# tensorflow/recommenders

Measured on NVIDIA H100. Metric: queries/sec brute-force top-K (1Mx64 candidates), higher is better.
Workload: dtype f32 (fp16 wgmma screening, fp32 accumulate + exact fp32 re-scoring)

## Files before the change

### include/tfrs_b200.h

```cpp
#ifndef TFRS_B200_H_
#define TFRS_B200_H_

#include <stddef.h>
#include <stdint.h>

#ifdef __cplusplus
extern "C" {
#endif

#define TFRS_B200_VERSION 102

enum {
  TFRS_OK = 0,
  TFRS_ERR_INVALID_ARG = -1,
  TFRS_ERR_UNSUPPORTED = -2,
  TFRS_ERR_CUDA = -3,
  TFRS_ERR_WORKSPACE_TOO_SMALL = -4,
  TFRS_ERR_NCCL = -5
};

enum { TFRS_I32 = 0, TFRS_I64 = 1 };

int tfrs_version(void);
const char* tfrs_last_error(void);
// ... 26 lines not shown
                           void* stream);

int tfrs_topk_exclude_rerank_f32(const float* scores, const int64_t* idx, int64_t Q, int k_fetched,
                                 const int64_t* identifiers, const int64_t* exclusions, int n_excl, int k_out,
                                 float* out_scores, int64_t* out_idx, void* stream);

int tfrs_count_above_f32(const float* scores, int64_t ld, int k, const float* positive_scores, int64_t Q,
                         int32_t* out_count, void* stream);

int tfrs_topk_hits_accumulate(const int32_t* count, const float* positive_scores, const float* sample_weight, int64_t Q,
                              const int32_t* ks, int n_ks, double* acc, void* stream);

int tfrs_topk_tc_layout(int64_t Q, int64_t N, int d, int k, int64_t* out10);

int tfrs_topk_tc_retry_layout(int64_t Q, int64_t N, int d, int k, int64_t* out4);

int tfrs_profile_enable(int on);
int tfrs_profile_read(float* stage_ms, int* calls);

int tfrs_topk_merge_strided(const float* scores, const int64_t* idx, int64_t list_stride_scores,
                            int64_t list_stride_idx, int n_lists, int64_t Q, int k_in, int k_out,
                            float* out_scores, int64_t* out_idx, void* stream);

int tfrs_topk_merge_sorted_strided(const float* scores, const int64_t* idx, int64_t list_stride_scores,
                                   int64_t list_stride_idx, int n_lists, int64_t Q, int k_in, int k_out,
                                   float* out_scores, int64_t* out_idx, void* stream);

typedef struct tfrs_comm* tfrs_comm_t;
int tfrs_comm_unique_id(void* out128);
int tfrs_comm_create(tfrs_comm_t* comm, int rank, int world, const void* unique_id128);
// ... 235 lines not shown
```

### recommenders_b200/_ffi.py

```python
from __future__ import annotations

import ctypes
import os
from typing import Optional

import torch

_HERE = os.path.dirname(os.path.abspath(__file__))
LIB_PATH = os.environ.get("TFRS_B200_LIB", os.path.join(_HERE, "libtfrs_b200.so"))

_lib: Optional[ctypes.CDLL] = None

I32, I64, BYTES = 0, 1, 2
c_p = ctypes.c_void_p
c_i = ctypes.c_int
c_l = ctypes.c_int64
c_f = ctypes.c_float
c_sz = ctypes.c_size_t
c_u32 = ctypes.c_uint32

_SIGNATURES = {
    "tfrs_version": (c_i, []),
    "tfrs_last_error": (ctypes.c_char_p, []),
    "tfrs_launch_count": (c_l, []),
    "tfrs_gather_f32": (c_i, [c_p, c_p, c_p, c_i, c_p, c_i, c_l, c_p, c_l, c_p, c_p]),
    "tfrs_topk_scan_workspace_bytes": (c_sz, [c_l, c_l, c_i, c_i]),
    "tfrs_topk_scan_f32": (c_i, [c_p, c_l, c_p, c_l, c_i, c_i, c_l, c_p, c_p, c_i, c_p, c_p, c_p, c_sz, c_p]),
    "tfrs_index_bytes": (c_sz, [c_l, c_i]),
    "tfrs_index_build": (c_i, [c_p, c_l, c_i, c_p, c_sz, c_p]),
    "tfrs_topk_tc_workspace_bytes": (c_sz, [c_l, c_l, c_i, c_i]),
    "tfrs_topk_tc_f32": (c_i, [c_p, c_l, c_p, c_p, c_l, c_i, c_i, c_l, c_p, c_p, c_p, c_sz, c_p]),
    "tfrs_topk_tc_exclude_f32": (c_i, [c_p, c_l, c_p, c_p, c_l, c_i, c_i, c_l, c_p, c_p, c_i, c_p, c_p, c_p, c_sz, c_p]),
    "tfrs_topk_tc_count_f32": (c_i, [c_p, c_l, c_p, c_p, c_l, c_i, c_i, c_p, c_p, c_p, c_sz, c_p]),
    "tfrs_topk_exclude_rerank_f32": (c_i, [c_p, c_p, c_l, c_i, c_p, c_p, c_i, c_i, c_p, c_p, c_p]),
    "tfrs_count_above_f32": (c_i, [c_p, c_l, c_i, c_p, c_l, c_p, c_p]),
    "tfrs_topk_hits_accumulate": (c_i, [c_p, c_p, c_p, c_l, c_p, c_i, c_p, c_p]),
    "tfrs_topk_tc_layout": (c_i, [c_l, c_l, c_i, c_i, c_p]),
    "tfrs_topk_tc_retry_layout": (c_i, [c_l, c_l, c_i, c_i, c_p]),
    "tfrs_dot_interaction_out_dim": (c_i, [c_i, c_i, c_i]),
    "tfrs_dot_interaction_fwd_f32": (c_i, [c_p, c_l, c_i, c_i, c_i, c_i, c_p, c_p]),
    "tfrs_dot_interaction_bwd_f32": (c_i, [c_p, c_p, c_l, c_i, c_i, c_i, c_i, c_p, c_p]),
    "tfrs_profile_enable": (c_i, [c_i]),
    "tfrs_profile_read": (c_i, [c_p, c_p]),
    "tfrs_topk_merge_strided": (c_i, [c_p, c_p, c_l, c_l, c_i, c_l, c_i, c_i, c_p, c_p, c_p]),
    "tfrs_topk_merge_sorted_strided": (c_i, [c_p, c_p, c_l, c_l, c_i, c_l, c_i, c_i, c_p, c_p, c_p]),
    "tfrs_comm_unique_id": (c_i, [c_p]),
    "tfrs_comm_create": (c_i, [c_p, c_i, c_i, c_p]),
    "tfrs_comm_destroy": (c_i, [c_p]),
    "tfrs_comm_enable_p2p": (c_i, [c_p, c_l, c_i]),
    "tfrs_comm_p2p_capacity": (c_i, [c_p, c_l, c_i]),
    "tfrs_comm_set_option": (c_i, [c_p, c_i, c_i]),
    "tfrs_comm_rank": (c_i, [c_p]),
    "tfrs_comm_world": (c_i, [c_p]),
# ... 165 lines not shown
```

### recommenders_b200/csrc/topk_tc.cu

```cuda
#include <cuda_fp16.h>
#include <math.h>
#include <stdlib.h>
#include <type_traits>
#include "rowselect.cuh"
#include "tc_ptx.cuh"

namespace tfrs {
namespace tc {

constexpr int TILE_N = 128;
constexpr int TILE_M = 128;
constexpr int QBLK = 256;
constexpr int KSLAB = 64;
constexpr int SLAB_BYTES = TILE_N * 128;
constexpr int HEADER_BYTES = 1024;
constexpr int THREADS = 512;
constexpr int CONSUMER_WARPS = 16;
constexpr int CAND_CAP = 2048;
constexpr int MAX_SAMPLE_STRIDE = 4;
constexpr int FIN_MAX_PARTS = 2 * 132;
constexpr int MAX_BINS = 1024;
constexpr int FP16_TARGET = 15;
constexpr float E_REL = 0.00108f;
constexpr float E_ACC = 0.00013f;

struct SideStats {
  unsigned int max_norm2_bits;
  unsigned int amax_bits;
  int exp;
  int pad;
};
struct IndexHeader {
  SideStats st;
  int d, d_pad, kb, pad;
  long long n, n_tiles;
};

__device__ __forceinline__ int rescale_exp(float amax) {
  int x = 0;
  if (!(amax > 0.f) || !(amax < INFINITY)) return 0;
  (void)frexpf(amax, &x);
  return FP16_TARGET - x;
}

__global__ void __launch_bounds__(256)
tile_image_kernel(const float* __restrict__ src, long long rows, int d, int kb, long long n_tiles,
                  const SideStats* __restrict__ st, unsigned char* __restrict__ img) {
  const int scale_exp = st->exp;
  const long long total = n_tiles * TILE_N * (long long)kb * 8;
  for (long long e = (long long)blockIdx.x * 256 + threadIdx.x; e < total; e += (long long)gridDim.x * 256) {
    int chunk = (int)(e % (kb * 8));
    long long row = e / (kb * 8);
    int slab = chunk / 8, cj = chunk % 8;
    int r = (int)(row % TILE_N);
    long long tile = row / TILE_N;
    int k0 = slab * KSLAB + cj * 8;
    __align__(16) __half v[8];
#pragma unroll
    for (int j = 0; j < 8; ++j) {
      float f = (row < rows && k0 + j < d) ? src[row * d + k0 + j] : 0.f;
      v[j] = __float2half_rn(ldexpf(f, scale_exp));
    }
    unsigned char* dst = img + tile * ((long long)kb * SLAB_BYTES) + (long long)slab * SLAB_BYTES + r * 128 + ((cj ^ (r & 7)) * 16);
    *reinterpret_cast<uint4*>(dst) = *reinterpret_cast<const uint4*>(v);
  }
}

template <int PASS>
__global__ void __launch_bounds__(256)
corpus_stats_kernel(const float* __restrict__ src, long long rows, int d, SideStats* __restrict__ st) {
  const int lane = threadIdx.x & 31;
  const long long warp = ((long long)blockIdx.x * 256 + threadIdx.x) >> 5;
  const long long nwarps = ((long long)gridDim.x * 256) >> 5;
  const int e = PASS ? st->exp : 0;
  float best = 0.f;
  for (long long row = warp; row < rows; row += nwarps) {
    const float* p = src + row * d;
    float acc = 0.f;
    for (int k = lane; k < d; k += 32) {
      const float x = p[k];
      if (PASS) { const float y = ldexpf(x, e); acc = fmaf(y, y, acc); } else acc = fmaxf(acc, fabsf(x));
    }
#pragma unroll
    for (int o = 16; o > 0; o >>= 1) {
      const float other = __shfl_xor_sync(0xffffffffu, acc, o);
      acc = PASS ? acc + other : fmaxf(acc, other);
    }
    best = fmaxf(best, acc);
  }
  if (lane == 0 && best > 0.f) {
    if (PASS) atomicMax(&st->max_norm2_bits, __float_as_uint(best * 1.0001f));
    else atomicMax(&st->amax_bits, __float_as_uint(best));
  }
}
__global__ void side_exp_kernel(SideStats* st) { st->exp = rescale_exp(__uint_as_float(st->amax_bits)); }
__global__ void header_kernel(IndexHeader* dst, IndexHeader h) { *dst = h; }

__global__ void __launch_bounds__(256)
tc_qprep_kernel(const float* __restrict__ q, long long Q, long long Qp, int d, int kb, const IndexHeader* __restrict__ hdr,
                unsigned char* __restrict__ qimg, float* __restrict__ margin, float* __restrict__ cut, int* __restrict__ qexp) {
  const int lane = threadIdx.x & 31;
  const long long row = ((long long)blockIdx.x * 256 + threadIdx.x) >> 5;
  if (row >= Qp) return;
  const bool real = row < Q;
  const float* p = q + row * d;
  float a = 0.f;
  if (real) for (int k = lane; k < d; k += 32) a = fmaxf(a, fabsf(p[k]));
#pragma unroll
  for (int o = 16; o > 0; o >>= 1) a = fmaxf(a, __shfl_xor_sync(0xffffffffu, a, o));
  const int e = rescale_exp(a);
  float n2 = 0.f;
// ... 29 lines not shown
enum { FILTER_FULL = 0, FILTER_NO_EMIT = 1, FILTER_NO_EPILOGUE = 2 };
#if defined(TFRS_DEBUG_SWITCHES) && defined(TFRS_FILTER_ABLATION)
constexpr int FILTER_ABLATION = TFRS_FILTER_ABLATION;
#else
constexpr int FILTER_ABLATION = FILTER_FULL;
#endif

struct ScanParams {
  const unsigned char* qimg;
  const unsigned char* cimg;
  long long Q, N;
  int nqb, parts, n_seq, stride;
  long long n_tiles;
  float* binmax; int bins_ld;
  int group, bins_per_part;
  const float* thr;
  const unsigned int* retry;
  unsigned int* count;
  float* cand_s;
  unsigned int* cand_i;
  int cap_part;
};

template <int KB, int STAGES, int MODE>
__global__ void __launch_bounds__(THREADS, 1)
tc_scan_kernel(const ScanParams p) {
  extern __shared__ __align__(1024) unsigned char smem_raw[];
  unsigned char* smem = reinterpret_cast<unsigned char*>((reinterpret_cast<uintptr_t>(smem_raw) + 1023) & ~uintptr_t(1023));
  unsigned char* sA = smem;
  unsigned char* sB = smem + 2 * KB * SLAB_BYTES;
  uint64_t* bars = reinterpret_cast<uint64_t*>(sB + STAGES * KB * SLAB_BYTES);
  uint64_t* full = bars;
  uint64_t* empty = bars + STAGES;
  uint64_t* a_full = bars + 2 * STAGES;

  const int wg = threadIdx.x >> 7, warp = (threadIdx.x >> 5) & 3, lane = threadIdx.x & 31;
  const int qb = blockIdx.x % p.nqb, part = blockIdx.x / p.nqb;
  const int u_begin = (int)((long long)part * p.n_seq / p.parts);
  const int u_end = (int)((long long)(part + 1) * p.n_seq / p.parts);
  const int n_iter = u_end - u_begin;
  const bool issuer = threadIdx.x == 0;
  auto rescanned = [&](long long row) { return p.retry == nullptr || (row < p.Q && p.retry[row] != 0u); };
  if (MODE == MODE_FILTER && p.retry != nullptr &&
      !__syncthreads_or(threadIdx.x < QBLK && rescanned((long long)qb * QBLK + threadIdx.x)))
    return;

  if (issuer) {
    for (int s = 0; s < STAGES; ++s) { mbar_init(&full[s], 1); mbar_init(&empty[s], CONSUMER_WARPS); }
    mbar_init(a_full, 1);
    asm volatile("fence.mbarrier_init.release.cluster;" ::: "memory");
  }
  __syncthreads();

  auto load_tile = [&](int it, int stage) {
    const long long tile = (long long)(u_begin + it) * p.stride;
    mbar_expect_tx(&full[stage], KB * SLAB_BYTES);
    if (MODE == MODE_FILTER)
      bulk_g2s_hint(sB + stage * KB * SLAB_BYTES, p.cimg + tile * ((long long)KB * SLAB_BYTES), KB * SLAB_BYTES, &full[stage],
                    l2_policy_evict_first());
    else
      bulk_g2s(sB + stage * KB * SLAB_BYTES, p.cimg + tile * ((long long)KB * SLAB_BYTES), KB * SLAB_BYTES, &full[stage]);
  };
  if (issuer) {
    mbar_expect_tx(a_full, 2 * KB * SLAB_BYTES);
    bulk_g2s(sA, p.qimg + (long long)qb * 2 * KB * SLAB_BYTES, 2 * KB * SLAB_BYTES, a_full);
    for (int it = 0; it < STAGES && it < n_iter; ++it) load_tile(it, it);
  }

  const long long row_a = (long long)qb * QBLK + wg * 64 + warp * 16 + (lane >> 2);
  const bool quad_leader = (lane & 3) == 0;
  float thr[2] = {INFINITY, INFINITY};
  if (MODE == MODE_FILTER) {
#pragma unroll
    for (int rr = 0; rr < 2; ++rr) if (row_a + 8 * rr < p.Q) thr[rr] = rescanned(row_a + 8 * rr) ? p.thr[row_a + 8 * rr] : NAN;
  }
  const unsigned int cap = (unsigned int)p.cap_part;
// ... 24 lines not shown
          wgmma_m64n64_rs(acc, afrag[k4], b_desc + (uint64_t)(k4 * 2), (uint32_t)(k4 != 0));
        else
          wgmma_m64n64_ss(acc, make_smem_desc(a0 + kb * SLAB_BYTES) + (uint64_t)(k4 * 2), b_desc + (uint64_t)(k4 * 2),
                          (uint32_t)((kb | k4) != 0));
      }
    }
    wgmma_commit();
  };
  auto epilogue = [&](const float (&acc)[32], long long col0, int it, auto half) {
    constexpr int H = decltype(half)::value;
    if (MODE != MODE_FILTER) {
#pragma unroll
      for (int j = 0; j < 8; ++j)
#pragma unroll
        for (int rr = 0; rr < 2; ++rr) binm[2 * rr + H] = max3(binm[2 * rr + H], acc[4 * j + 2 * rr], acc[4 * j + 2 * rr + 1]);
      if (H == 1 && (++in_group == p.group || it == n_iter - 1)) {
#pragma unroll
        for (int s = 0; s < 4; ++s) {
          const float m = quad_max(binm[s]);
          const long long row = row_a + 8 * (s >> 1);
          if (quad_leader && row < p.Q)
            p.binmax[row * p.bins_ld + (long long)part * p.bins_per_part * 2 + (s & 1) + 2 * bin_out] = m;
          binm[s] = -INFINITY;
        }
        ++bin_out; in_group = 0;
      }
    } else {
      if (FILTER_ABLATION == FILTER_NO_EPILOGUE) {
#pragma unroll
        for (int i = 0; i < 32; ++i) sink ^= __float_as_uint(acc[i]);
        return;
      }
      float pm[2][8];
      bool pass = false;
#pragma unroll
      for (int rr = 0; rr < 2; ++rr) {
#pragma unroll
// ... 34 lines not shown
              ++cnt[s];
            } else {
              ovf |= 1u << s;
            }
          }
        }
      }
    }
  };

  float acc0[32], acc1[32];
  int stage = 0; uint32_t phase = 0;
  int prev_stage = 0; uint32_t prev_phase = 0;
  auto tile_step = [&](int it, auto last_tile) {
    constexpr bool LAST = decltype(last_tile)::value;
    const long long col0 = (long long)(u_begin + it) * p.stride * TILE_N;
    issue(acc1, stage, 1);
    epilogue(acc0, col0, it, std::integral_constant<int, 0>{});
    const int next_stage = stage + 1 == STAGES ? 0 : stage + 1;
    const uint32_t next_phase = stage + 1 == STAGES ? phase ^ 1 : phase;
    if (!LAST) {
      mbar_wait(&full[next_stage], next_phase);
      issue(acc0, next_stage, 0);
      wgmma_wait<1>();
    } else {
      wgmma_wait<0>();
    }
    acc_fence(acc1);
    __syncwarp();
    if (lane == 0) mbar_arrive(&empty[stage]);
    if (!LAST && issuer && it >= 1 && it - 1 + STAGES < n_iter) {
// ... 9 lines not shown
    }
  };
  if (n_iter > 0) {
    mbar_wait(&full[0], 0);
    issue(acc0, 0, 0);
    wgmma_wait<0>();
    acc_fence(acc0);
    for (int it = 0; it + 1 < n_iter; ++it) tile_step(it, std::false_type{});
    tile_step(n_iter - 1, std::true_type{});
  }
  if (MODE == MODE_SAMPLE) {
#pragma unroll
    for (int s = 0; s < 4; ++s) {
      const long long row = row_a + 8 * (s >> 1);
      if (quad_leader && row < p.Q)
        for (int b = bin_out; b < p.bins_per_part; ++b)
          p.binmax[row * p.bins_ld + (long long)part * p.bins_per_part * 2 + (s & 1) + 2 * b] = -INFINITY;
    }
  } else if (quad_leader) {
#pragma unroll
    for (int s = 0; s < 4; ++s)
      if (rescanned(row_a + 8 * (s >> 1)))
        p.count[((row_a + 8 * (s >> 1)) * p.parts + part) * 2 + (s & 1)] =
            FILTER_ABLATION != FILTER_FULL ? sink : ((ovf >> s) & 1u) ? (cap + 1u) : cnt[s];
  }
}

__device__ __forceinline__ unsigned int f2key(float f) {
  unsigned int u = __float_as_uint(f);
  return (u & 0x80000000u) ? ~u : (u | 0x80000000u);
}
__device__ __forceinline__ float key2f(unsigned int k) {
  return __uint_as_float((k & 0x80000000u) ? (k & 0x7fffffffu) : ~k);
}
__device__ __forceinline__ unsigned long long rank_key(float s, unsigned int idx) {
  const unsigned int lo = (0xFFFFFFFEu - 2u * idx) | (__float_as_uint(s) == 0x80000000u ? 1u : 0u);
  return ((unsigned long long)f2key(s + 0.0f) << 32) | lo;
}
__device__ __forceinline__ float rank_key_score(unsigned long long e) {
  return __uint_as_float(__float_as_uint(key2f((unsigned int)(e >> 32))) | ((unsigned int)e << 31));
// ... 17 lines not shown
  }
  return prefix;
}
__device__ __forceinline__ unsigned int warp_kth_largest_smem(const unsigned int* keys, int n, int k, int lane, unsigned int prefix, int top_bit) {
  for (int bit = top_bit; bit >= 0; --bit) {
    const unsigned int cand = prefix | (1u << bit);
    int c = 0;
    for (int t = lane; t < n; t += 32) c += (keys[t] >= cand) ? 1 : 0;
    c = __reduce_add_sync(0xffffffffu, c);
    if (c >= k) prefix = cand;
  }
  return prefix;
}

template <int KPL>
__global__ void __launch_bounds__(256)
tc_threshold_kernel(const float* __restrict__ binmax, int bins_ld, int n_bins, int k, int k_filter, const float* __restrict__ margin,
                    float* __restrict__ thr, float* __restrict__ thr_safe, unsigned int* __restrict__ overflow,
                    unsigned int* __restrict__ retry, long long Q) {
  const int lane = threadIdx.x & 31;
  const long long row = ((long long)blockIdx.x * 256 + threadIdx.x) >> 5;
  if (row >= Q) return;
  const float* src = binmax + row * bins_ld;
  unsigned int key[KPL];
#pragma unroll
  for (int j = 0; j < KPL; ++j) { const int i = j * 32 + lane; key[j] = i < n_bins ? f2key(__ldg(src + i)) : 0u; }
  const float safe = key2f(warp_kth_largest_regs<KPL>(key, k)) - margin[row];
  const float filter = k_filter < k ? key2f(warp_kth_largest_regs<KPL>(key, k_filter)) - margin[row] : safe;
  if (lane == 0) { thr[row] = filter; thr_safe[row] = safe; overflow[row] = 0; retry[row] = 0; }
}

enum { FIN_TOPK = 0, FIN_EXCLUDE = 1, FIN_COUNT = 2 };
constexpr int FW_WARPS = 4;

struct FinParams {
  const float* q; const float* corpus; int d; int k; long long index_offset; long long N; long long Q;
  const unsigned int* count; const float* cand_s; const unsigned int* cand_i; int segs; int cap_part;
  const float* cut; float* thr; const float* thr_safe; unsigned int* overflow;
  unsigned int* retry; int retry_pass;
  int cap_keys, cap_band;
  unsigned int* band_idx; int* band_n;
  int allow_short;
  float* out_s; long long* out_i;
  const long long* identifiers; const long long* exclusions; int n_excl; int k_out;
// ... 416 lines not shown
static void prof_mark(cudaStream_t st, int stage) {
  if (!g_prof.on || g_prof.calls >= Prof::MAXC) return;
  int c = g_prof.calls;
  while (g_prof.created <= c) {
    for (int s = 0; s <= Prof::STAGES_; ++s) cudaEventCreate(&g_prof.ev[g_prof.created][s]);
    ++g_prof.created;
  }
  cudaEventRecord(g_prof.ev[c][stage], st);
  if (stage == Prof::STAGES_) ++g_prof.calls;
}

struct Plan {
  int kb, stages; long long n_tiles; int nqb; long long Qp;
  int stride, n_sample, group, bins_per_part, n_bins, bins_ld, parts_sample, parts_full, cap_part, cap_keys, cap_band;
  int k_filter;
  size_t smem;
  size_t o_qimg, o_margin, o_cut, o_thr, o_qexp, o_count, o_ovf, o_binmax, o_cand, o_tmp, o_band, o_bandn, o_thr_safe, o_retry,
      total;
};

static int filter_bin_rank(int k, int stride) {
  if (stride <= 1 || k <= 1) return k;
  const int n = k - 1;
  const double p = 1.0 / stride;
  double tail = 0.0;
  for (int r = n; r >= 1; --r) {
    tail += exp(lgamma(n + 1.0) - lgamma(r + 1.0) - lgamma(n - r + 1.0) + r * log(p) + (n - r) * log1p(-p));
    if (tail > 1e-9) return r + 1;
  }
  return 1;
// ... 18 lines not shown
  pl.n_sample = (int)ceil_div(full_tiles, pl.stride);
  if (2ll * pl.n_sample < 4ll * k) return false;
  const int sms = sm_count();
  int parts = sms / pl.nqb; if (parts < 1) parts = 1; if (parts > FIN_MAX_PARTS / 2) parts = FIN_MAX_PARTS / 2;
  pl.parts_sample = parts < pl.n_sample ? parts : pl.n_sample;
  pl.parts_full = (long long)parts < pl.n_tiles ? parts : (int)pl.n_tiles;
  {
    const int iters_max = (int)ceil_div(pl.n_sample, pl.parts_sample);
    const int target = 4 * k > 512 ? 4 * k : 512;
    int g = 1;
    while ((long long)pl.parts_sample * ceil_div(iters_max, g) * 2 > target && g < iters_max) ++g;
    pl.group = g;
    pl.bins_per_part = (int)ceil_div(iters_max, g);
    pl.n_bins = pl.parts_sample * pl.bins_per_part * 2;
    if (pl.n_bins > MAX_BINS || pl.n_bins < 2 * k) return false;
    pl.bins_ld = (pl.n_bins + 31) / 32 * 32;
  }
  {
    const double lambda = (double)k * pl.stride / (pl.parts_full * 2.0);
    const double want = 2.0 * lambda + 12.0 * sqrt(lambda) + 8.0;
    int p2 = 32; while (p2 < want && p2 < 512) p2 <<= 1;
    pl.cap_part = p2;
    int ck = 1024; while (ck < 1.6 * 1.3 * k * pl.stride && ck < 4096) ck <<= 1;
    pl.cap_keys = ck;
    pl.cap_band = ck / 2;
  }
  pl.smem = (size_t)(2 + pl.stages) * pl.kb * SLAB_BYTES + 1024  + 256 ;
  size_t o = 0;
  auto take = [&](size_t bytes) { size_t r = o; o += align_up(bytes, 1024); return r; };
  pl.o_qimg = take((size_t)pl.nqb * 2 * pl.kb * SLAB_BYTES);
  pl.o_margin = take((size_t)pl.Qp * 4);
// ... 89 lines not shown
  unsigned int* cand_i = (unsigned int*)(w + pl.o_cand + (size_t)pl.Qp * pl.parts_full * 2 * pl.cap_part * 32);
  float* tmp_s = (float*)(w + pl.o_tmp);
  long long* tmp_i = (long long*)(w + pl.o_tmp + align_up((size_t)c.Q * c.k * 4, 8));
  float* thr_safe = (float*)(w + pl.o_thr_safe);
  unsigned int* retry = (unsigned int*)(w + pl.o_retry);
  const IndexHeader* hdr = (const IndexHeader*)c.index_buf;
  const unsigned char* cimg = (const unsigned char*)c.index_buf + HEADER_BYTES;
  const int k_filter = (c.mode == FIN_COUNT || c.hook) ? c.k : pl.k_filter;

  prof_mark(st, 0);
  tc_qprep_kernel<<<(unsigned)ceil_div(pl.Qp * 32, 256), 256, 0, st>>>(c.q, c.Q, pl.Qp, c.d, pl.kb, hdr, qimg, margin, cut, qexp);
  TFRS_LAUNCH_CHECK();
  ScanParams sp{};
  sp.qimg = qimg; sp.cimg = cimg; sp.Q = c.Q; sp.N = c.N; sp.nqb = pl.nqb; sp.n_tiles = pl.n_tiles;
  sp.binmax = binmax; sp.bins_ld = pl.bins_ld; sp.group = pl.group; sp.bins_per_part = pl.bins_per_part;
  sp.thr = thr; sp.count = count; sp.cand_s = cand_s; sp.cand_i = cand_i; sp.cap_part = pl.cap_part;
  prof_mark(st, 1);
  int rc = launch_scan_mode(pl, sp, st, MODE_SAMPLE);
  if (rc) return rc;
  if (pl.n_bins <= 512)
    tc_threshold_kernel<16><<<(unsigned)ceil_div(c.Q * 32, 256), 256, 0, st>>>(binmax, pl.bins_ld, pl.n_bins, c.k, k_filter, margin,
                                                                                 thr, thr_safe, ovf, retry, c.Q);
  else
    tc_threshold_kernel<32><<<(unsigned)ceil_div(c.Q * 32, 256), 256, 0, st>>>(binmax, pl.bins_ld, pl.n_bins, c.k, k_filter, margin,
                                                                                 thr, thr_safe, ovf, retry, c.Q);
  TFRS_LAUNCH_CHECK();
  if (c.hook) {
    rc = c.hook(c.hook_ctx, thr, margin, cut, qexp, &hdr->st.exp, c.Q, st);
    if (rc) return rc;
  }
  prof_mark(st, 2);
  rc = launch_scan_mode(pl, sp, st, MODE_FILTER);
  if (rc) return rc;
  prof_mark(st, 3);
  if (FILTER_ABLATION != FILTER_FULL) { prof_mark(st, 4); return TFRS_OK; }
  FinParams fp{};
  fp.q = c.q; fp.corpus = c.corpus; fp.d = c.d; fp.k = c.k; fp.index_offset = c.index_offset; fp.N = c.N; fp.Q = c.Q;
  fp.count = count; fp.cand_s = cand_s; fp.cand_i = cand_i; fp.segs = pl.parts_full * 2; fp.cap_part = pl.cap_part;
  fp.cut = cut; fp.thr = thr; fp.thr_safe = thr_safe; fp.overflow = ovf; fp.retry = retry; fp.out_s = c.out_s; fp.out_i = c.out_i;
  fp.cap_keys = pl.cap_keys; fp.cap_band = pl.cap_band; fp.allow_short = c.allow_short;
// ... 22 lines not shown
    }
  }
  prof_mark(st, 4);
  return TFRS_OK;
}

}
}

using namespace tfrs;
using namespace tfrs::tc;

extern "C" size_t tfrs_index_bytes(int64_t N, int d) {
  if (N <= 0 || d <= 0 || d > 128) return 0;
  int kb = (d + KSLAB - 1) / KSLAB;
  return (size_t)HEADER_BYTES + (size_t)ceil_div(N, TILE_N) * kb * SLAB_BYTES;
}

extern "C" int tfrs_index_build(const float* corpus, int64_t N, int d, void* index_buf, size_t index_bytes, void* stream) {
  TFRS_CHECK_ARG(corpus && index_buf && N > 0 && d > 0, "index_build: bad arguments");
  if (d > 128) { set_error("index_build: d=%d > 128 is not supported by the tensor-core path", d); return TFRS_ERR_UNSUPPORTED; }
  TFRS_CHECK_ARG(index_bytes >= tfrs_index_bytes(N, d), "index_build: buffer too small");
  TFRS_CHECK_ARG((reinterpret_cast<uintptr_t>(index_buf) & 15) == 0, "index_build: buffer must be 16-byte aligned");
  cudaStream_t st = (cudaStream_t)stream;
  IndexHeader h{};
  h.d = d; h.kb = (d + KSLAB - 1) / KSLAB; h.d_pad = h.kb * KSLAB; h.n = N; h.n_tiles = ceil_div(N, TILE_N);
  TFRS_CUDA(cudaMemsetAsync(index_buf, 0, HEADER_BYTES, st));
  header_kernel<<<1, 1, 0, st>>>(reinterpret_cast<IndexHeader*>(index_buf), h);
  TFRS_LAUNCH_CHECK();
  SideStats* cst = &reinterpret_cast<IndexHeader*>(index_buf)->st;
  const unsigned sgrid = (unsigned)(sm_count() * 8);
  corpus_stats_kernel<0><<<sgrid, 256, 0, st>>>(corpus, N, d, cst);
  TFRS_LAUNCH_CHECK();
  side_exp_kernel<<<1, 1, 0, st>>>(cst);
  TFRS_LAUNCH_CHECK();
  corpus_stats_kernel<1><<<sgrid, 256, 0, st>>>(corpus, N, d, cst);
  TFRS_LAUNCH_CHECK();
  long long chunks = h.n_tiles * TILE_N * (long long)h.kb * 8;
  unsigned blocks = (unsigned)(ceil_div(chunks, 256) < (1 << 20) ? ceil_div(chunks, 256) : (1 << 20));
  tile_image_kernel<<<blocks, 256, 0, st>>>(corpus, N, d, h.kb, h.n_tiles, cst, (unsigned char*)index_buf + HEADER_BYTES);
  TFRS_LAUNCH_CHECK();
  return TFRS_OK;
}

extern "C" size_t tfrs_topk_tc_workspace_bytes(int64_t Q, int64_t N, int d, int k) {
  Plan pl;
  if (!make_plan(Q, N, d, k, pl)) return 0;
  return pl.total + 16;
}

extern "C" int tfrs_topk_tc_f32(const float* q, int64_t Q, const float* corpus, const void* index_buf, int64_t N, int d,
                                int k, int64_t index_offset, float* out_scores, int64_t* out_idx, void* ws, size_t ws_bytes,
                                void* stream) {
  TFRS_CHECK_ARG(q && corpus && index_buf && out_scores && out_idx, "topk_tc: NULL pointer");
  TFRS_CHECK_ARG(k <= N, "input must have at least k columns. Had %lld, needed %d", (long long)N, k);
  Call c{};
  c.mode = FIN_TOPK; c.q = q; c.Q = Q; c.corpus = corpus; c.index_buf = index_buf; c.N = N; c.d = d; c.k = k;
// ... 44 lines not shown
  if (!make_plan(Q, N, d, k, pl)) { set_error("topk_tc_layout: unsupported shape"); return TFRS_ERR_UNSUPPORTED; }
  out10[0] = (int64_t)pl.o_count; out10[1] = (int64_t)pl.o_ovf; out10[2] = (int64_t)pl.o_thr; out10[3] = (int64_t)pl.o_cand;
  out10[4] = pl.parts_full * 2; out10[5] = pl.cap_part; out10[6] = pl.Qp; out10[7] = (int64_t)pl.o_cut;
  out10[8] = pl.n_bins; out10[9] = (int64_t)pl.o_qexp;
  return TFRS_OK;
}

extern "C" int tfrs_topk_tc_retry_layout(int64_t Q, int64_t N, int d, int k, int64_t* out4) {
  TFRS_CHECK_ARG(out4, "topk_tc_retry_layout: NULL pointer");
  Plan pl;
  if (!make_plan(Q, N, d, k, pl)) { set_error("topk_tc_retry_layout: unsupported shape"); return TFRS_ERR_UNSUPPORTED; }
  out4[0] = (int64_t)pl.o_thr_safe; out4[1] = (int64_t)pl.o_retry; out4[2] = pl.k_filter; out4[3] = pl.stride;
  return TFRS_OK;
}

extern "C" int tfrs_profile_enable(int on) {
  g_prof.on = on != 0;
  g_prof.calls = 0;
  return TFRS_OK;
}

extern "C" int tfrs_profile_read(float* stage_ms, int* calls) {
  TFRS_CHECK_ARG(stage_ms && calls, "profile_read: NULL pointer");
  TFRS_CUDA(cudaDeviceSynchronize());
  for (int s = 0; s < 4; ++s) stage_ms[s] = 0.f;
  for (int c = 0; c < g_prof.calls; ++c)
    for (int s = 0; s < 4; ++s) {
      float ms = 0.f;
      TFRS_CUDA(cudaEventElapsedTime(&ms, g_prof.ev[c][s], g_prof.ev[c][s + 1]));
      stage_ms[s] += ms;
// ... 5 lines not shown
```

Baseline: 3.069 million.

## Add norm-based sample tile image for tighter top-K threshold estimation

At index build time, the code selects the top-norm N/8 corpus rows using a radix select and stores them as an extra tile image. It checks with a Gaussian tail estimate and probe queries whether high-norm rows dominate the nearest neighbours. When the check passes, the sampling scan reads this dense high-norm subset instead of strided tiles, which should give higher per-query thresholds and fewer candidates in the filter pass. The cost is a larger index, a much more expensive build with dozens of extra kernel launches, and threshold quality that depends on the data distribution.

After: 3.242 million (median of 6 runs). 1.06x the previous value.

```diff
diff --git a/include/tfrs_b200.h b/include/tfrs_b200.h
--- a/include/tfrs_b200.h
+++ b/include/tfrs_b200.h
@@ -64,6 +64,8 @@
 int tfrs_topk_tc_layout(int64_t Q, int64_t N, int d, int k, int64_t* out10);
 
 int tfrs_topk_tc_retry_layout(int64_t Q, int64_t N, int d, int k, int64_t* out4);
+
+int tfrs_topk_tc_sample_layout(int64_t Q, int64_t N, int d, int k, int64_t* out8);
 
 int tfrs_profile_enable(int on);
 int tfrs_profile_read(float* stage_ms, int* calls);
diff --git a/recommenders_b200/_ffi.py b/recommenders_b200/_ffi.py
--- a/recommenders_b200/_ffi.py
+++ b/recommenders_b200/_ffi.py
@@ -37,6 +37,7 @@
     "tfrs_topk_hits_accumulate": (c_i, [c_p, c_p, c_p, c_l, c_p, c_i, c_p, c_p]),
     "tfrs_topk_tc_layout": (c_i, [c_l, c_l, c_i, c_i, c_p]),
     "tfrs_topk_tc_retry_layout": (c_i, [c_l, c_l, c_i, c_i, c_p]),
+    "tfrs_topk_tc_sample_layout": (c_i, [c_l, c_l, c_i, c_i, c_p]),
     "tfrs_dot_interaction_out_dim": (c_i, [c_i, c_i, c_i]),
     "tfrs_dot_interaction_fwd_f32": (c_i, [c_p, c_l, c_i, c_i, c_i, c_i, c_p, c_p]),
     "tfrs_dot_interaction_bwd_f32": (c_i, [c_p, c_p, c_l, c_i, c_i, c_i, c_i, c_p, c_p]),
diff --git a/recommenders_b200/csrc/topk_tc.cu b/recommenders_b200/csrc/topk_tc.cu
--- a/recommenders_b200/csrc/topk_tc.cu
+++ b/recommenders_b200/csrc/topk_tc.cu
@@ -30,11 +30,23 @@
   int exp;
   int pad;
 };
+enum { SAMPLE_STRIDED = 0, SAMPLE_NORM = 1 };
+constexpr long long NORM_SAMPLE_MIN_N = 1ll << 19;
+constexpr int NORM_SAMPLE_DIV = 8;
+constexpr double NORM_SAMPLE_TAIL = 1e-4;
+constexpr double NORM_SAMPLE_MIN_PHI = 0.35;
+constexpr int NORM_PROBES = 256, NORM_PROBE_K = 100;
+constexpr float NORM_PROBE_MIN_MEAN = 0.35f, NORM_PROBE_MIN_EACH = 0.25f;
 struct IndexHeader {
   SideStats st;
-  int d, d_pad, kb, pad;
+  int d, d_pad, kb, sample;
   long long n, n_tiles;
+  float phi;
+  float probe_mean, probe_min;
 };
+__host__ __device__ inline long long norm_sample_tiles(long long N) {
+  return N >= NORM_SAMPLE_MIN_N && N < (1ll << 31) ? N / NORM_SAMPLE_DIV / 128 : 0;
+}
 
 __device__ __forceinline__ int rescale_exp(float amax) {
   int x = 0;
@@ -45,7 +57,7 @@
 
 __global__ void __launch_bounds__(256)
 tile_image_kernel(const float* __restrict__ src, long long rows, int d, int kb, long long n_tiles,
-                  const SideStats* __restrict__ st, unsigned char* __restrict__ img) {
+                  const SideStats* __restrict__ st, unsigned char* __restrict__ img, const int* __restrict__ rowmap) {
   const int scale_exp = st->exp;
   const long long total = n_tiles * TILE_N * (long long)kb * 8;
   for (long long e = (long long)blockIdx.x * 256 + threadIdx.x; e < total; e += (long long)gridDim.x * 256) {
@@ -55,10 +67,11 @@
     int r = (int)(row % TILE_N);
     long long tile = row / TILE_N;
     int k0 = slab * KSLAB + cj * 8;
+    const long long srow = (rowmap != nullptr && row < rows) ? (long long)rowmap[row] : row;
     __align__(16) __half v[8];
 #pragma unroll
     for (int j = 0; j < 8; ++j) {
-      float f = (row < rows && k0 + j < d) ? src[row * d + k0 + j] : 0.f;
+      float f = (row < rows && k0 + j < d) ? src[srow * d + k0 + j] : 0.f;
       v[j] = __float2half_rn(ldexpf(f, scale_exp));
     }
     unsigned char* dst = img + tile * ((long long)kb * SLAB_BYTES) + (long long)slab * SLAB_BYTES + r * 128 + ((cj ^ (r & 7)) * 16);
@@ -68,7 +81,8 @@
 
 template <int PASS>
 __global__ void __launch_bounds__(256)
-corpus_stats_kernel(const float* __restrict__ src, long long rows, int d, SideStats* __restrict__ st) {
+corpus_stats_kernel(const float* __restrict__ src, long long rows, int d, SideStats* __restrict__ st,
+                    unsigned int* __restrict__ norm2_key = nullptr) {
   const int lane = threadIdx.x & 31;
   const long long warp = ((long long)blockIdx.x * 256 + threadIdx.x) >> 5;
   const long long nwarps = ((long long)gridDim.x * 256) >> 5;
@@ -86,6 +100,7 @@
       const float other = __shfl_xor_sync(0xffffffffu, acc, o);
       acc = PASS ? acc + other : fmaxf(acc, other);
     }
+    if (PASS && norm2_key != nullptr && lane == 0) norm2_key[row] = __float_as_uint(acc);
     best = fmaxf(best, acc);
   }
   if (lane == 0 && best > 0.f) {
@@ -95,6 +110,159 @@
 }
 __global__ void side_exp_kernel(SideStats* st) { st->exp = rescale_exp(__uint_as_float(st->amax_bits)); }
 __global__ void header_kernel(IndexHeader* dst, IndexHeader h) { *dst = h; }
+
+struct NormSelect {
+  unsigned long long cnt[32];
+  long long need;
+  double lo, hi;
+};
+constexpr int NS_CHUNK = 8192;
+
+__device__ __forceinline__ unsigned int norm_select_prefix(const NormSelect* s, long long S, int lowest) {
+  unsigned int prefix = 0u;
+  for (int b = 31; b > lowest; --b)
+    if (s->cnt[b] >= (unsigned long long)S) prefix |= 1u << b;
+  return prefix;
+}
+
+__global__ void __launch_bounds__(256)
+norm_select_count_kernel(const unsigned int* __restrict__ key, long long n, long long S, int bit, NormSelect* s) {
+  const unsigned int cand = norm_select_prefix(s, S, bit) | (1u << bit);
+  unsigned int c = 0;
+  for (long long i = (long long)blockIdx.x * 256 + threadIdx.x; i < n; i += (long long)gridDim.x * 256) c += key[i] >= cand ? 1u : 0u;
+  c = __reduce_add_sync(0xffffffffu, c);
+  if ((threadIdx.x & 31) == 0 && c) atomicAdd(&s->cnt[bit], (unsigned long long)c);
+}
+
+__global__ void __launch_bounds__(256)
+norm_select_chunks_kernel(const unsigned int* __restrict__ key, long long n, long long S, const NormSelect* s, int* __restrict__ blk) {
+  __shared__ int sh[2];
+  const unsigned int T = norm_select_prefix(s, S, -1);
+  if (threadIdx.x == 0) { sh[0] = 0; sh[1] = 0; }
+  __syncthreads();
+  int gt = 0, eq = 0;
+  const long long r0 = (long long)blockIdx.x * NS_CHUNK;
+  for (int t = threadIdx.x; t < NS_CHUNK; t += 256) {
+    const long long i = r0 + t;
+    if (i < n) { gt += key[i] > T ? 1 : 0; eq += key[i] == T ? 1 : 0; }
+  }
+  gt = __reduce_add_sync(0xffffffffu, gt); eq = __reduce_add_sync(0xffffffffu, eq);
+  if ((threadIdx.x & 31) == 0) { atomicAdd(&sh[0], gt); atomicAdd(&sh[1], eq); }
+  __syncthreads();
+  if (threadIdx.x == 0) { blk[2 * blockIdx.x] = sh[0]; blk[2 * blockIdx.x + 1] = sh[1]; }
+}
+
+__global__ void norm_select_offsets_kernel(int* __restrict__ blk, int nblk, long long S, NormSelect* s) {
+  long long gt = 0;
+  for (int b = 0; b < nblk; ++b) gt += blk[2 * b];
+  const long long need = S - gt;
+  long long sel = 0, eq = 0;
+  for (int b = 0; b < nblk; ++b) {
+    const long long g = blk[2 * b], e = blk[2 * b + 1];
+    const long long take = need - eq < 0 ? 0 : (need - eq < e ? need - eq : e);
+    blk[2 * b] = (int)sel; blk[2 * b + 1] = (int)eq;
+    sel += g + take; eq += e;
+  }
+  s->need = need;
+}
+
+__global__ void __launch_bounds__(256)
+norm_select_write_kernel(const unsigned int* __restrict__ key, long long n, long long S, const NormSelect* s,
+                         const int* __restrict__ blk, int* __restrict__ rowlist) {
+  __shared__ int wsel[8], weq[8];
+  const unsigned int T = norm_select_prefix(s, S, -1);
+  const long long need = s->need;
+  const int warp = threadIdx.x >> 5, lane = threadIdx.x & 31;
+  const unsigned int lt = (1u << lane) - 1u;
+  int sel_base = blk[2 * blockIdx.x], eq_base = blk[2 * blockIdx.x + 1];
+  const long long r0 = (long long)blockIdx.x * NS_CHUNK;
+  for (int t0 = 0; t0 < NS_CHUNK; t0 += 256) {
+    const long long i = r0 + t0 + threadIdx.x;
+    const unsigned int k = i < n ? key[i] : 0u;
+    const bool is_eq = i < n && k == T;
+    const unsigned int veq = __ballot_sync(0xffffffffu, is_eq);
+    if (lane == 0) weq[warp] = __popc(veq);
+    __syncthreads();
+    int eq_before = eq_base, eq_all = 0;
+    for (int w = 0; w < 8; ++w) { eq_before += w < warp ? weq[w] : 0; eq_all += weq[w]; }
+    eq_before += __popc(veq & lt);
+    const bool is_sel = i < n && (k > T || (is_eq && eq_before < need));
+    const unsigned int vsel = __ballot_sync(0xffffffffu, is_sel);
+    if (lane == 0) wsel[warp] = __popc(vsel);
+    __syncthreads();
+    int sel_before = sel_base, sel_all = 0;
+    for (int w = 0; w < 8; ++w) { sel_before += w < warp ? wsel[w] : 0; sel_all += wsel[w]; }
+    if (is_sel) rowlist[sel_before + __popc(vsel & lt)] = (int)i;
+    sel_base += sel_all; eq_base += eq_all;
+    __syncthreads();
+  }
+}
+
+__device__ __forceinline__ double norm_tail(unsigned int norm2_key, double t) {
+  const double r = sqrt((double)__uint_as_float(norm2_key));
+  return r > 0.0 ? 0.5 * erfc(t / (r * 1.4142135623730951)) : 0.0;
+}
+__global__ void __launch_bounds__(256)
+norm_phi_partial_kernel(const unsigned int* __restrict__ key, const int* __restrict__ rows, long long n, const NormSelect* s,
+                        double* __restrict__ partial) {
+  __shared__ double sh[256];
+  const double t = 0.5 * (s->lo + s->hi);
+  double acc = 0.0;
+  const long long r0 = (long long)blockIdx.x * NS_CHUNK;
+  for (int u = threadIdx.x; u < NS_CHUNK; u += 256) {
+    const long long j = r0 + u;
+    if (j < n) acc += norm_tail(key[rows ? (long long)rows[j] : j], t);
+  }
+  sh[threadIdx.x] = acc;
+  __syncthreads();
+  for (int o = 128; o > 0; o >>= 1) {
+    if (threadIdx.x < o) sh[threadIdx.x] += sh[threadIdx.x + o];
+    __syncthreads();
+  }
+  if (threadIdx.x == 0) partial[blockIdx.x] = sh[0];
+}
+__global__ void norm_phi_step_kernel(const double* __restrict__ partial, int nblk, long long N, int final, NormSelect* s,
+                                     IndexHeader* hdr, const float* __restrict__ share) {
+  double sum = 0.0;
+  for (int b = 0; b < nblk; ++b) sum += partial[b];
+  const double target = (double)N * NORM_SAMPLE_TAIL;
+  if (!final) {
+    const double t = 0.5 * (s->lo + s->hi);
+    if (sum > target) s->lo = t; else s->hi = t;
+  } else {
+    const double phi = sum / target;
+    float mean = 0.f, mn = 1.f;
+    for (int i = 0; i < NORM_PROBES; ++i) { mean += share[i]; mn = fminf(mn, share[i]); }
+    mean /= NORM_PROBES;
+    hdr->phi = (float)phi; hdr->probe_mean = mean; hdr->probe_min = mn;
+    hdr->sample = phi >= NORM_SAMPLE_MIN_PHI && mean >= NORM_PROBE_MIN_MEAN && mn >= NORM_PROBE_MIN_EACH ? SAMPLE_NORM : SAMPLE_STRIDED;
+  }
+}
+
+__global__ void norm_probe_gather_kernel(const float* __restrict__ corpus, long long N, int d, float* __restrict__ probes) {
+  const int pr = blockIdx.x;
+  const long long row = (long long)pr * N / NORM_PROBES;
+  for (int t = threadIdx.x; t < d; t += 32) probes[(long long)pr * d + t] = corpus[row * d + t];
+}
+__global__ void norm_sample_flags_kernel(const int* __restrict__ rowlist, long long S, unsigned char* __restrict__ in_sample) {
+  for (long long j = (long long)blockIdx.x * 256 + threadIdx.x; j < S; j += (long long)gridDim.x * 256) in_sample[rowlist[j]] = 1;
+}
+__global__ void norm_probe_share_kernel(const long long* __restrict__ idx, long long N, const unsigned char* __restrict__ in_sample,
+                                        float* __restrict__ share) {
+  const int pr = blockIdx.x, lane = threadIdx.x;
+  const long long self = (long long)pr * N / NORM_PROBES;
+  int hit = 0, n = 0;
+  for (int j = lane; j < NORM_PROBE_K + 1; j += 32) {
+    const long long i = idx[(long long)pr * (NORM_PROBE_K + 1) + j];
+    if (i != self && i >= 0 && i < N) { ++n; hit += in_sample[i]; }
+  }
+  hit = __reduce_add_sync(0xffffffffu, hit); n = __reduce_add_sync(0xffffffffu, n);
+  if (lane == 0) share[pr] = n > 0 ? (float)hit / (float)n : 0.f;
+}
+__global__ void norm_phi_init_kernel(NormSelect* s, const SideStats* st) {
+  s->lo = 0.0;
+  s->hi = 40.0 * sqrt((double)__uint_as_float(st->max_norm2_bits)) + 1e-30;
+}
 
 __global__ void __launch_bounds__(256)
 tc_qprep_kernel(const float* __restrict__ q, long long Q, long long Qp, int d, int kb, const IndexHeader* __restrict__ hdr,
@@ -154,6 +322,9 @@
   long long n_tiles;
   float* binmax; int bins_ld;
   int group, bins_per_part;
+  const IndexHeader* hdr;
+  const unsigned char* simg;
+  int n_seq_norm, group_norm, bins_per_part_norm;
   const float* thr;
   const unsigned int* retry;
   unsigned int* count;
@@ -162,9 +333,8 @@
   int cap_part;
 };
 
-template <int KB, int STAGES, int MODE>
-__global__ void __launch_bounds__(THREADS, 1)
-tc_scan_kernel(const ScanParams p) {
+template <int KB, int STAGES, int MODE, bool NORM>
+__device__ __forceinline__ void tc_scan_body(const ScanParams& p) {
   extern __shared__ __align__(1024) unsigned char smem_raw[];
   unsigned char* smem = reinterpret_cast<unsigned char*>((reinterpret_cast<uintptr_t>(smem_raw) + 1023) & ~uintptr_t(1023));
   unsigned char* sA = smem;
@@ -176,8 +346,11 @@
 
   const int wg = threadIdx.x >> 7, warp = (threadIdx.x >> 5) & 3, lane = threadIdx.x & 31;
   const int qb = blockIdx.x % p.nqb, part = blockIdx.x / p.nqb;
-  const int u_begin = (int)((long long)part * p.n_seq / p.parts);
-  const int u_end = (int)((long long)(part + 1) * p.n_seq / p.parts);
+  const unsigned char* const cimg = NORM ? p.simg : p.cimg;
+  const int n_seq = NORM ? p.n_seq_norm : p.n_seq, stride = NORM ? 1 : p.stride;
+  const int group = NORM ? p.group_norm : p.group, bins_per_part = NORM ? p.bins_per_part_norm : p.bins_per_part;
+  const int u_begin = (int)((long long)part * n_seq / p.parts);
+  const int u_end = (int)((long long)(part + 1) * n_seq / p.parts);
   const int n_iter = u_end - u_begin;
   const bool issuer = threadIdx.x == 0;
   auto rescanned = [&](long long row) { return p.retry == nullptr || (row < p.Q && p.retry[row] != 0u); };
@@ -193,13 +366,13 @@
   __syncthreads();
 
   auto load_tile = [&](int it, int stage) {
-    const long long tile = (long long)(u_begin + it) * p.stride;
+    const long long tile = (long long)(u_begin + it) * stride;
     mbar_expect_tx(&full[stage], KB * SLAB_BYTES);
     if (MODE == MODE_FILTER)
-      bulk_g2s_hint(sB + stage * KB * SLAB_BYTES, p.cimg + tile * ((long long)KB * SLAB_BYTES), KB * SLAB_BYTES, &full[stage],
+      bulk_g2s_hint(sB + stage * KB * SLAB_BYTES, cimg + tile * ((long long)KB * SLAB_BYTES), KB * SLAB_BYTES, &full[stage],
                     l2_policy_evict_first());
     else
-      bulk_g2s(sB + stage * KB * SLAB_BYTES, p.cimg + tile * ((long long)KB * SLAB_BYTES), KB * SLAB_BYTES, &full[stage]);
+      bulk_g2s(sB + stage * KB * SLAB_BYTES, cimg + tile * ((long long)KB * SLAB_BYTES), KB * SLAB_BYTES, &full[stage]);
   };
   if (issuer) {
     mbar_expect_tx(a_full, 2 * KB * SLAB_BYTES);
@@ -254,13 +427,13 @@
       for (int j = 0; j < 8; ++j)
 #pragma unroll
         for (int rr = 0; rr < 2; ++rr) binm[2 * rr + H] = max3(binm[2 * rr + H], acc[4 * j + 2 * rr], acc[4 * j + 2 * rr + 1]);
-      if (H == 1 && (++in_group == p.group || it == n_iter - 1)) {
+      if (H == 1 && (++in_group == group || it == n_iter - 1)) {
 #pragma unroll
         for (int s = 0; s < 4; ++s) {
           const float m = quad_max(binm[s]);
           const long long row = row_a + 8 * (s >> 1);
           if (quad_leader && row < p.Q)
-            p.binmax[row * p.bins_ld + (long long)part * p.bins_per_part * 2 + (s & 1) + 2 * bin_out] = m;
+            p.binmax[row * p.bins_ld + (long long)part * bins_per_part * 2 + (s & 1) + 2 * bin_out] = m;
           binm[s] = -INFINITY;
         }
         ++bin_out; in_group = 0;
@@ -325,7 +498,7 @@
   int prev_stage = 0; uint32_t prev_phase = 0;
   auto tile_step = [&](int it, auto last_tile) {
     constexpr bool LAST = decltype(last_tile)::value;
-    const long long col0 = (long long)(u_begin + it) * p.stride * TILE_N;
+    const long long col0 = (long long)(u_begin + it) * stride * TILE_N;
     issue(acc1, stage, 1);
     epilogue(acc0, col0, it, std::integral_constant<int, 0>{});
     const int next_stage = stage + 1 == STAGES ? 0 : stage + 1;
@@ -365,8 +538,8 @@
     for (int s = 0; s < 4; ++s) {
       const long long row = row_a + 8 * (s >> 1);
       if (quad_leader && row < p.Q)
-        for (int b = bin_out; b < p.bins_per_part; ++b)
-          p.binmax[row * p.bins_ld + (long long)part * p.bins_per_part * 2 + (s & 1) + 2 * b] = -INFINITY;
+        for (int b = bin_out; b < bins_per_part; ++b)
+          p.binmax[row * p.bins_ld + (long long)part * bins_per_part * 2 + (s & 1) + 2 * b] = -INFINITY;
     }
   } else if (quad_leader) {
 #pragma unroll
@@ -375,6 +548,15 @@
         p.count[((row_a + 8 * (s >> 1)) * p.parts + part) * 2 + (s & 1)] =
             FILTER_ABLATION != FILTER_FULL ? sink : ((ovf >> s) & 1u) ? (cap + 1u) : cnt[s];
   }
+}
+
+template <int KB, int STAGES, int MODE>
+__global__ void __launch_bounds__(THREADS, 1)
+tc_scan_kernel(const __grid_constant__ ScanParams p) {
+  if constexpr (MODE == MODE_SAMPLE) {
+    if (p.simg != nullptr && p.hdr->sample == SAMPLE_NORM) { tc_scan_body<KB, STAGES, MODE, true>(p); return; }
+  }
+  tc_scan_body<KB, STAGES, MODE, false>(p);
 }
 
 __device__ __forceinline__ unsigned int f2key(float f) {
@@ -422,13 +604,9 @@
 }
 
 template <int KPL>
-__global__ void __launch_bounds__(256)
-tc_threshold_kernel(const float* __restrict__ binmax, int bins_ld, int n_bins, int k, int k_filter, const float* __restrict__ margin,
-                    float* __restrict__ thr, float* __restrict__ thr_safe, unsigned int* __restrict__ overflow,
-                    unsigned int* __restrict__ retry, long long Q) {
-  const int lane = threadIdx.x & 31;
-  const long long row = ((long long)blockIdx.x * 256 + threadIdx.x) >> 5;
-  if (row >= Q) return;
+__device__ __forceinline__ void thresholds_of_row(const float* __restrict__ binmax, int bins_ld, int n_bins, int k, int k_filter,
+                                                  const float* __restrict__ margin, float* __restrict__ thr, float* __restrict__ thr_safe,
+                                                  unsigned int* __restrict__ overflow, unsigned int* __restrict__ retry, long long row, int lane) {
   const float* src = binmax + row * bins_ld;
   unsigned int key[KPL];
 #pragma unroll
@@ -436,6 +614,18 @@
   const float safe = key2f(warp_kth_largest_regs<KPL>(key, k)) - margin[row];
   const float filter = k_filter < k ? key2f(warp_kth_largest_regs<KPL>(key, k_filter)) - margin[row] : safe;
   if (lane == 0) { thr[row] = filter; thr_safe[row] = safe; overflow[row] = 0; retry[row] = 0; }
+}
+template <int KPL>
+__global__ void __launch_bounds__(256)
+tc_threshold_kernel(const float* __restrict__ binmax, int bins_ld, int n_bins, int k, int k_filter, const float* __restrict__ margin,
+                    float* __restrict__ thr, float* __restrict__ thr_safe, unsigned int* __restrict__ overflow,
+                    unsigned int* __restrict__ retry, long long Q, const IndexHeader* __restrict__ hdr, int n_bins_norm) {
+  const int lane = threadIdx.x & 31;
+  const long long row = ((long long)blockIdx.x * 256 + threadIdx.x) >> 5;
+  if (row >= Q) return;
+  if (n_bins_norm > 0 && hdr->sample == SAMPLE_NORM) { n_bins = n_bins_norm; k_filter = k; }
+  if (KPL > 16 && n_bins <= 512) thresholds_of_row<16>(binmax, bins_ld, n_bins, k, k_filter, margin, thr, thr_safe, overflow, retry, row, lane);
+  else thresholds_of_row<KPL>(binmax, bins_ld, n_bins, k, k_filter, margin, thr, thr_safe, overflow, retry, row, lane);
 }
 
 enum { FIN_TOPK = 0, FIN_EXCLUDE = 1, FIN_COUNT = 2 };
@@ -882,6 +1072,7 @@
   int kb, stages; long long n_tiles; int nqb; long long Qp;
   int stride, n_sample, group, bins_per_part, n_bins, bins_ld, parts_sample, parts_full, cap_part, cap_keys, cap_band;
   int k_filter;
+  int n_seq_norm, group_norm, bins_per_part_norm, n_bins_norm;
   size_t smem;
   size_t o_qimg, o_margin, o_cut, o_thr, o_qexp, o_count, o_ovf, o_binmax, o_cand, o_tmp, o_band, o_bandn, o_thr_safe, o_retry,
       total;
@@ -930,7 +1121,18 @@
     pl.bins_per_part = (int)ceil_div(iters_max, g);
     pl.n_bins = pl.parts_sample * pl.bins_per_part * 2;
     if (pl.n_bins > MAX_BINS || pl.n_bins < 2 * k) return false;
-    pl.bins_ld = (pl.n_bins + 31) / 32 * 32;
+    pl.n_seq_norm = (int)norm_sample_tiles(N);
+    pl.group_norm = pl.bins_per_part_norm = pl.n_bins_norm = 0;
+    if (pl.n_seq_norm >= pl.parts_sample) {
+      const int iters_norm = (int)ceil_div(pl.n_seq_norm, pl.parts_sample);
+      int gn = 1;
+      while ((long long)pl.parts_sample * ceil_div(iters_norm, gn) * 2 > MAX_BINS) ++gn;
+      const int bpp = (int)ceil_div(iters_norm, gn);
+      if (pl.parts_sample * bpp * 2 >= 4 * k) { pl.group_norm = gn; pl.bins_per_part_norm = bpp; pl.n_bins_norm = pl.parts_sample * bpp * 2; }
+    }
+    if (pl.n_bins_norm == 0) pl.n_seq_norm = 0;
+    const int bins_max = pl.n_bins > pl.n_bins_norm ? pl.n_bins : pl.n_bins_norm;
+    pl.bins_ld = (bins_max + 31) / 32 * 32;
   }
   {
     const double lambda = (double)k * pl.stride / (pl.parts_full * 2.0);
@@ -1050,16 +1252,19 @@
   ScanParams sp{};
   sp.qimg = qimg; sp.cimg = cimg; sp.Q = c.Q; sp.N = c.N; sp.nqb = pl.nqb; sp.n_tiles = pl.n_tiles;
   sp.binmax = binmax; sp.bins_ld = pl.bins_ld; sp.group = pl.group; sp.bins_per_part = pl.bins_per_part;
+  sp.hdr = hdr;
+  sp.simg = pl.n_bins_norm > 0 ? cimg + pl.n_tiles * pl.kb * (long long)SLAB_BYTES : nullptr;
+  sp.n_seq_norm = pl.n_seq_norm; sp.group_norm = pl.group_norm; sp.bins_per_part_norm = pl.bins_per_part_norm;
   sp.thr = thr; sp.count = count; sp.cand_s = cand_s; sp.cand_i = cand_i; sp.cap_part = pl.cap_part;
   prof_mark(st, 1);
   int rc = launch_scan_mode(pl, sp, st, MODE_SAMPLE);
   if (rc) return rc;
-  if (pl.n_bins <= 512)
+  if (pl.n_bins <= 512 && pl.n_bins_norm <= 512)
     tc_threshold_kernel<16><<<(unsigned)ceil_div(c.Q * 32, 256), 256, 0, st>>>(binmax, pl.bins_ld, pl.n_bins, c.k, k_filter, margin,
-                                                                                 thr, thr_safe, ovf, retry, c.Q);
+                                                                                 thr, thr_safe, ovf, retry, c.Q, hdr, pl.n_bins_norm);
   else
     tc_threshold_kernel<32><<<(unsigned)ceil_div(c.Q * 32, 256), 256, 0, st>>>(binmax, pl.bins_ld, pl.n_bins, c.k, k_filter, margin,
-                                                                                 thr, thr_safe, ovf, retry, c.Q);
+                                                                                 thr, thr_safe, ovf, retry, c.Q, hdr, pl.n_bins_norm);
   TFRS_LAUNCH_CHECK();
   if (c.hook) {
     rc = c.hook(c.hook_ctx, thr, margin, cut, qexp, &hdr->st.exp, c.Q, st);
@@ -1112,7 +1317,7 @@
 extern "C" size_t tfrs_index_bytes(int64_t N, int d) {
   if (N <= 0 || d <= 0 || d > 128) return 0;
   int kb = (d + KSLAB - 1) / KSLAB;
-  return (size_t)HEADER_BYTES + (size_t)ceil_div(N, TILE_N) * kb * SLAB_BYTES;
+  return (size_t)HEADER_BYTES + (size_t)(ceil_div(N, TILE_N) + norm_sample_tiles(N)) * kb * SLAB_BYTES;
 }
 
 extern "C" int tfrs_index_build(const float* corpus, int64_t N, int d, void* index_buf, size_t index_bytes, void* stream) {
@@ -1132,13 +1337,92 @@
   TFRS_LAUNCH_CHECK();
   side_exp_kernel<<<1, 1, 0, st>>>(cst);
   TFRS_LAUNCH_CHECK();
-  corpus_stats_kernel<1><<<sgrid, 256, 0, st>>>(corpus, N, d, cst);
+  const long long s_tiles = norm_sample_tiles(N);
+  if (s_tiles == 0) {
+    corpus_stats_kernel<1><<<sgrid, 256, 0, st>>>(corpus, N, d, cst);
+    TFRS_LAUNCH_CHECK();
+  }
+  auto image = [&](long long rows, long long tiles, unsigned char* dst, const int* rowmap) {
+    const long long chunks = tiles * TILE_N * (long long)h.kb * 8;
+    const unsigned blocks = (unsigned)(ceil_div(chunks, 256) < (1 << 20) ? ceil_div(chunks, 256) : (1 << 20));
+    tile_image_kernel<<<blocks, 256, 0, st>>>(corpus, rows, d, h.kb, tiles, cst, dst, rowmap);
+  };
+  unsigned char* img = (unsigned char*)index_buf + HEADER_BYTES;
+  image(N, h.n_tiles, img, nullptr);
   TFRS_LAUNCH_CHECK();
-  long long chunks = h.n_tiles * TILE_N * (long long)h.kb * 8;
-  unsigned blocks = (unsigned)(ceil_div(chunks, 256) < (1 << 20) ? ceil_div(chunks, 256) : (1 << 20));
-  tile_image_kernel<<<blocks, 256, 0, st>>>(corpus, N, d, h.kb, h.n_tiles, cst, (unsigned char*)index_buf + HEADER_BYTES);
-  TFRS_LAUNCH_CHECK();
-  return TFRS_OK;
+  if (s_tiles == 0) return TFRS_OK;
+
+  const long long S = s_tiles * TILE_N;
+  const int nblk = (int)ceil_div(N, NS_CHUNK), nblk_s = (int)ceil_div(S, NS_CHUNK);
+  const size_t o_rows = align_up((size_t)N * 4, 256), o_blk = o_rows + align_up((size_t)S * 4, 256);
+  const size_t o_part = o_blk + align_up((size_t)nblk * 8, 256), o_sel = o_part + align_up((size_t)nblk * 8, 256);
+  Plan ppl;
+  const bool probe_ok = make_plan(NORM_PROBES, N, d, NORM_PROBE_K + 1, ppl);
+  const size_t pk = (size_t)NORM_PROBES * (NORM_PROBE_K + 1);
+  const size_t o_probe = o_sel + align_up(sizeof(NormSelect), 256), o_ps = o_probe + align_up((size_t)NORM_PROBES * d * 4, 256);
+  const size_t o_pi = o_ps + align_up(pk * 4, 256), o_share = o_pi + align_up(pk * 8, 256);
+  const size_t o_flag = o_share + align_up((size_t)NORM_PROBES * 4, 256), o_pws = o_flag + align_up((size_t)N, 256);
+  const size_t ws_bytes = probe_ok ? ppl.total + 16 : 0;
+  unsigned char* scratch = nullptr;
+  TFRS_CUDA(cudaMallocAsync((void**)&scratch, o_pws + ws_bytes, st));
+  unsigned int* key = (unsigned int*)scratch;
+  int* rowlist = (int*)(scratch + o_rows);
+  int* blk = (int*)(scratch + o_blk);
+  double* partial = (double*)(scratch + o_part);
+  NormSelect* sel = (NormSelect*)(scratch + o_sel);
+  int rc = TFRS_OK;
+  auto launched = [&]() {
+    count_launch();
+    const cudaError_t e = cudaGetLastError();
+    if (e != cudaSuccess && rc == TFRS_OK) { set_error("index_build: %s", cudaGetErrorString(e)); rc = TFRS_ERR_CUDA; }
+  };
+  if (cudaMemsetAsync(sel, 0, sizeof(NormSelect), st) != cudaSuccess) { set_error("index_build: memset failed"); rc = TFRS_ERR_CUDA; }
+  corpus_stats_kernel<1><<<sgrid, 256, 0, st>>>(corpus, N, d, cst, key);
+  launched();
+  for (int bit = 31; bit >= 0; --bit) { norm_select_count_kernel<<<sgrid, 256, 0, st>>>(key, N, S, bit, sel); launched(); }
+  norm_select_chunks_kernel<<<nblk, 256, 0, st>>>(key, N, S, sel, blk);
+  launched();
+  norm_select_offsets_kernel<<<1, 1, 0, st>>>(blk, nblk, S, sel);
+  launched();
+  norm_select_write_kernel<<<nblk, 256, 0, st>>>(key, N, S, sel, blk, rowlist);
+  launched();
+  image(S, s_tiles, img + h.n_tiles * h.kb * (long long)SLAB_BYTES, rowlist);
+  launched();
+  norm_phi_init_kernel<<<1, 1, 0, st>>>(sel, cst);
+  launched();
+  IndexHeader* hdr = reinterpret_cast<IndexHeader*>(index_buf);
+  for (int it = 0; it < 48; ++it) {
+    norm_phi_partial_kernel<<<nblk, 256, 0, st>>>(key, nullptr, N, sel, partial);
+    launched();
+    norm_phi_step_kernel<<<1, 1, 0, st>>>(partial, nblk, N, 0, sel, hdr, nullptr);
+    launched();
+  }
+  float* share = (float*)(scratch + o_share);
+  if (cudaMemsetAsync(share, 0, (size_t)NORM_PROBES * 4, st) != cudaSuccess && rc == TFRS_OK) { set_error("index_build: memset failed"); rc = TFRS_ERR_CUDA; }
+  if (probe_ok && rc == TFRS_OK) {
+    unsigned char* flags = scratch + o_flag;
+    if (cudaMemsetAsync(flags, 0, (size_t)N, st) != cudaSuccess) { set_error("index_build: memset failed"); rc = TFRS_ERR_CUDA; }
+    norm_sample_flags_kernel<<<sgrid, 256, 0, st>>>(rowlist, S, flags);
+    launched();
+    float* probes = (float*)(scratch + o_probe);
+    norm_probe_gather_kernel<<<NORM_PROBES, 32, 0, st>>>(corpus, N, d, probes);
+    launched();
+    Call c{};
+    c.mode = FIN_TOPK; c.q = probes; c.Q = NORM_PROBES; c.corpus = corpus; c.index_buf = index_buf; c.N = N; c.d = d;
+    c.k = NORM_PROBE_K + 1; c.ws = scratch + o_pws; c.ws_bytes = ws_bytes; c.st = st;
+    c.out_s = (float*)(scratch + o_ps); c.out_i = (long long*)(scratch + o_pi);
+    const int prc = run_call(c);
+    if (prc != TFRS_OK && rc == TFRS_OK) rc = prc;
+    norm_probe_share_kernel<<<NORM_PROBES, 32, 0, st>>>(c.out_i, N, flags, share);
+    launched();
+  }
+  norm_phi_partial_kernel<<<nblk_s, 256, 0, st>>>(key, rowlist, S, sel, partial);
+  launched();
+  norm_phi_step_kernel<<<1, 1, 0, st>>>(partial, nblk_s, N, 1, sel, hdr, share);
+  launched();
+  const cudaError_t fe = cudaFreeAsync(scratch, st);
+  if (fe != cudaSuccess && rc == TFRS_OK) { set_error("index_build: %s", cudaGetErrorString(fe)); rc = TFRS_ERR_CUDA; }
+  return rc;
 }
 
 extern "C" size_t tfrs_topk_tc_workspace_bytes(int64_t Q, int64_t N, int d, int k) {
@@ -1213,6 +1497,15 @@
   return TFRS_OK;
 }
 
+extern "C" int tfrs_topk_tc_sample_layout(int64_t Q, int64_t N, int d, int k, int64_t* out8) {
+  TFRS_CHECK_ARG(out8, "topk_tc_sample_layout: NULL pointer");
+  Plan pl;
+  if (!make_plan(Q, N, d, k, pl)) { set_error("topk_tc_sample_layout: unsupported shape"); return TFRS_ERR_UNSUPPORTED; }
+  out8[0] = (int64_t)pl.o_binmax; out8[1] = pl.bins_ld; out8[2] = pl.n_bins_norm; out8[3] = pl.group_norm;
+  out8[4] = pl.bins_per_part_norm; out8[5] = pl.parts_sample; out8[6] = pl.n_seq_norm; out8[7] = (int64_t)pl.o_margin;
+  return TFRS_OK;
+}
+
 extern "C" int tfrs_profile_enable(int on) {
   g_prof.on = on != 0;
   g_prof.calls = 0;
```
